# yoshitomo-matsubara/sc2-benchmark

Hardware: AMD Instinct MI355X
Metric: images/s + bpp, Entropic-Student ResNet-50 224^2 (higher is better)
Workload: dtype bf16

## Files before the change

### sc2-benchmark_amd/csrc/conv1x1_pair.hip

```cpp
#include <stdlib.h>

#include <atomic>

#include "sc2_common.h"

#ifndef SC2_NT_PAIR
#define SC2_NT_PAIR 0
#endif

namespace {

typedef __attribute__((address_space(3))) void *lds_ptr_t;
typedef float f32x2_t __attribute__((ext_vector_type(2)));
typedef __bf16 bf16x2_t __attribute__((ext_vector_type(2)));
typedef unsigned u32x4_t __attribute__((ext_vector_type(4)));
__device__ __forceinline__ uint32_t pack2(f32x2_t v) {
    return __builtin_bit_cast(uint32_t, __builtin_convertvector(v, bf16x2_t));
}

#if defined(__HIP_DEVICE_COMPILE__)
typedef __amdgpu_buffer_rsrc_t buf_rsrc_t;
__device__ __forceinline__ buf_rsrc_t make_rsrc(const uint16_t *base, uint32_t bytes) {
    return __builtin_amdgcn_make_buffer_rsrc(const_cast<uint16_t *>(base), 0, (int)bytes, 0x00020000);
}
__device__ __forceinline__ void buf_load_lds16(buf_rsrc_t r, lds_ptr_t dst, uint32_t voff, uint32_t soff) {
    __builtin_amdgcn_raw_ptr_buffer_load_lds(r, dst, 16, (int)voff, (int)soff, 0, 0);
}
__device__ __forceinline__ uint4 buf_load16(buf_rsrc_t r, uint32_t voff, uint32_t soff) {
    return __builtin_bit_cast(uint4, __builtin_amdgcn_raw_buffer_load_b128(r, (int)voff, (int)soff, 0));
}
__device__ __forceinline__ void buf_store16(buf_rsrc_t r, uint32_t voff, uint32_t soff, u32x4_t v) {
    __builtin_amdgcn_raw_buffer_store_b128(v, r, (int)voff, (int)soff, SC2_NT_PAIR ? SC2_BUF_AUX_NT : 0);
    __builtin_amdgcn_sched_barrier(0);
    asm volatile("s_nop 1" ::: "memory");
    __builtin_amdgcn_sched_barrier(0);
}
#else
typedef int buf_rsrc_t;
__device__ __forceinline__ buf_rsrc_t make_rsrc(const uint16_t *, uint32_t) { return 0; }
__device__ __forceinline__ void buf_load_lds16(buf_rsrc_t, lds_ptr_t, uint32_t, uint32_t) {}
__device__ __forceinline__ uint4 buf_load16(buf_rsrc_t, uint32_t, uint32_t) { return make_uint4(0, 0, 0, 0); }
__device__ __forceinline__ void buf_store16(buf_rsrc_t, uint32_t, uint32_t, u32x4_t) {}
#endif

template <int OFF>
__device__ __forceinline__ u32x4_t lds_read16_imm(uint32_t addr) {
    u32x4_t v;
    asm volatile("ds_read_b128 %0, %1 offset:%2" : "=v"(v) : "v"(addr), "n"(OFF) : "memory");
    return v;
}
__device__ __forceinline__ void lds_write16(uint32_t addr, u32x4_t v) {
    asm volatile("ds_write_b128 %0, %1" ::"v"(addr), "v"(v) : "memory");
}

#ifndef SC2_PAIR_DBG
#define SC2_PAIR_DBG 0
#endif

struct PairArgs {
    const uint16_t *__restrict__ o;
    const uint16_t *__restrict__ w3;
    const float *__restrict__ b3;
    const uint16_t *__restrict__ idn;
    uint16_t *__restrict__ h;
    const uint16_t *__restrict__ w1;
    const float *__restrict__ b1;
    uint16_t *__restrict__ u;
    int M, n_tiles;
    int rev;
    unsigned *tile_ctr;
};

template <int C, int K1, int N2, int MT>
__global__ __launch_bounds__(512, 2) void conv1x1_pair_kernel(const PairArgs p) {
    constexpr int P = MT * 16;
    constexpr int KS1 = K1 / 32, KS2 = C / 32;
    constexpr int NT1 = C / 8 / 16;
    constexpr int ROWB = C * 2;
    constexpr int CPR = ROWB / 16;
    constexpr int IMG = P * ROWB, SLAB = P * 64, OT = KS1 * SLAB;
    constexpr int NT2 = N2 / 128;
    static_assert(N2 == 128 || N2 == 256, "one or two 16-channel tiles of u per wave");
    static_assert(N2 <= C, "the u staging lives in the image region");
    static_assert(CPR == 64, "one image row = one LDS-DMA wave-instruction");
    constexpr int UROW = N2 * 2, UCPR = UROW / 16;
    constexpr int OQ = (P * K1 * 2 / 16 + 511) / 512;
    constexpr int UQ = (P * UCPR + 511) / 512;
    constexpr int IQ = (P * CPR + 511) / 512;
    extern __shared__ __attribute__((aligned(16))) unsigned char smem[];
    unsigned char *img = smem;
    unsigned char *ot = smem + IMG;
    volatile int *next_slot = reinterpret_cast<volatile int *>(smem + IMG + OT);
    float *bias_lds = reinterpret_cast<float *>(smem + IMG + OT + 16);

    const uint32_t lds_base = (uint32_t)(uintptr_t)(lds_ptr_t)smem;
    const int tid = threadIdx.x, lane = tid & 63;
    const int wn = __builtin_amdgcn_readfirstlane(tid >> 6);

    constexpr uint32_t OOB = 0x80000000u;
    const buf_rsrc_t rs_idn = make_rsrc(p.idn, (uint32_t)((long long)p.M * ROWB));
    const buf_rsrc_t rs_o = make_rsrc(p.o, (uint32_t)((long long)p.M * K1 * 2));
    const buf_rsrc_t rs_h = make_rsrc(p.h, (uint32_t)((long long)p.M * ROWB));
    const buf_rsrc_t rs_u = make_rsrc(p.u, (uint32_t)((long long)p.M * N2 * 2));

    auto load_o = [&](int tile, uint4 (&ov)[OQ], int tq) {
        const bool t_ok = tile < p.n_tiles;
        const int tpos = p.rev ? p.n_tiles - 1 - tile : tile;
        const uint32_t so = (uint32_t)(t_ok ? (long long)tpos * P * (K1 * 2) : 0);
#pragma unroll
        for (int k = 0; k < OQ; ++k) {
            const int q = tq + 512 * k;
            const bool ok = t_ok && q < P * (K1 / 8) && (long long)tpos * P + q / (K1 / 8) < p.M;
            ov[k] = buf_load16(rs_o, ok ? (uint32_t)q * 16u : OOB, so);
        }
    };
    auto store_o = [&](const uint4 (&ov)[OQ], int tq) {
#pragma unroll
        for (int k = 0; k < OQ; ++k) {
            const int q = tq + 512 * k;
            if (q < P * (K1 / 8)) {
                const int row = q / (K1 / 8), c16 = q % (K1 / 8);
                lds_write16(lds_base + IMG + (c16 >> 2) * SLAB + row * 64 + (((c16 & 3) ^ ((row >> 1) & 3)) << 4),
                            __builtin_bit_cast(u32x4_t, ov[k]));
            }
        }
    };
    auto issue_identity = [&](int tile, int lq) {
        static_assert(P % 8 == 0, "every wave takes P / 8 rows: straight-line issue, exact vmcnt bookkeeping");
#pragma unroll
        for (int r = 0; r < P / 8; ++r) {
            const int row = wn + 8 * r;
            const long long m = (long long)(p.rev ? p.n_tiles - 1 - tile : tile) * P + row;
            const bool ok = tile < p.n_tiles && m < p.M && !(SC2_PAIR_DBG & 1);
            const uint32_t voff = ok ? (uint32_t)((lq ^ (row & 15)) << 4) : OOB;
            buf_load_lds16(rs_idn, (lds_ptr_t)(img + row * ROWB), voff, (uint32_t)(ok ? m * ROWB : 0));
        }
    };

    uint4 wv[KS1][NT1];
    const buf_rsrc_t rs_w3 = make_rsrc(p.w3, (uint32_t)(C * K1 * 2));
    const uint32_t w3_vo = (uint32_t)(((wn * NT1) * KS1 * 64 + lane) * 16);
    auto load_w = [&]() {
#pragma unroll
        for (int j = 0; j < NT1; ++j)
#pragma unroll
            for (int s = 0; s < KS1; ++s) wv[s][j] = buf_load16(rs_w3, w3_vo, (uint32_t)((j * KS1 + s) * 1024));
    };
    load_w();
    const buf_rsrc_t rs_w1 = make_rsrc(p.w1, (uint32_t)(N2 * C * 2));
    const uint32_t w1_vo = (uint32_t)(((wn * NT2) * KS2 * 64 + lane) * 16);

    for (int k = tid; k < C + N2; k += 512) bias_lds[k] = k < C ? p.b3[k] : p.b1[k - C];
    int tile = blockIdx.x;
    int next_tile = tile + gridDim.x;
    {
        uint4 ov[OQ];
        load_o(tile, ov, tid);
        store_o(ov, tid);
        issue_identity(tile, lane);
    }
    __syncthreads();

    bool first = true;
    while (tile < p.n_tiles) {
        const long long m0 = (long long)(p.rev ? p.n_tiles - 1 - tile : tile) * P;
        int tq = tid, lq = lane;
        asm volatile("" : "+v"(tq), "+v"(lq));
        const int frow = lq & 15, fq = lq >> 4;
        const int o_lane = frow * 64 + ((fq ^ ((frow >> 1) & 3)) << 4);
        const int img_row = frow * ROWB;
        unsigned claimed = 0;
        if (tid == 0) {
            const unsigned one = 1u;
            asm volatile("global_atomic_add %0, %1, %2, off sc0" : "=v"(claimed) : "v"(p.tile_ctr), "v"(one) : "memory");
        }
        f32x4_t acc[MT][NT1];
#pragma unroll
        for (int i = 0; i < MT; ++i)
#pragma unroll
            for (int j = 0; j < NT1; ++j) acc[i][j] = f32x4_t{0.f, 0.f, 0.f, 0.f};
        {
            const uint32_t o_addr = lds_base + IMG + o_lane;
#pragma unroll
            for (int s = 0; s < KS1; ++s) {
                u32x4_t xa[4], xb[3];
                static_assert(MT == 7, "the asm waits below name 4 + 3 registers");
                xa[0] = lds_read16_imm<0 * 1024>(o_addr + s * SLAB);
                xa[1] = lds_read16_imm<1 * 1024>(o_addr + s * SLAB);
                xa[2] = lds_read16_imm<2 * 1024>(o_addr + s * SLAB);
                xa[3] = lds_read16_imm<3 * 1024>(o_addr + s * SLAB);
                asm volatile("s_waitcnt lgkmcnt(0)" : "+v"(xa[0]), "+v"(xa[1]), "+v"(xa[2]), "+v"(xa[3])::"memory");
                xb[0] = lds_read16_imm<4 * 1024>(o_addr + s * SLAB);
                xb[1] = lds_read16_imm<5 * 1024>(o_addr + s * SLAB);
                xb[2] = lds_read16_imm<6 * 1024>(o_addr + s * SLAB);
#pragma unroll
                for (int i = 0; i < 4; ++i) {
                    const bf16x8_t xf = __builtin_bit_cast(bf16x8_t, xa[i]);
#pragma unroll
                    for (int j = 0; j < NT1; ++j)
                        acc[i][j] = __builtin_amdgcn_mfma_f32_16x16x32_bf16(__builtin_bit_cast(bf16x8_t, wv[s][j]), xf, acc[i][j], 0, 0, 0);
                }
                asm volatile("s_waitcnt lgkmcnt(0)" : "+v"(xb[0]), "+v"(xb[1]), "+v"(xb[2])::"memory");
#pragma unroll
                for (int i = 0; i < 3; ++i) {
                    const bf16x8_t xf = __builtin_bit_cast(bf16x8_t, xb[i]);
#pragma unroll
                    for (int j = 0; j < NT1; ++j)
                        acc[4 + i][j] = __builtin_amdgcn_mfma_f32_16x16x32_bf16(__builtin_bit_cast(bf16x8_t, wv[s][j]), xf, acc[4 + i][j], 0, 0, 0);
                }
                __builtin_amdgcn_sched_barrier(0);
            }
        }
        if (first) asm volatile("s_waitcnt vmcnt(0)" ::: "memory");
        else if (wn == 0) asm volatile("s_waitcnt vmcnt(%0)" ::"n"(IQ + UQ + 1) : "memory");
        else asm volatile("s_waitcnt vmcnt(%0)" ::"n"(IQ + UQ) : "memory");
        first = false;
        __syncthreads();
#pragma unroll
        for (int j = 0; j < NT1; ++j) {
            const int c16 = wn * (NT1 * 2) + j * 2 + (fq >> 1);
            const float4 b3v = *reinterpret_cast<const float4 *>(bias_lds + wn * (NT1 * 16) + j * 16 + fq * 4);
            const f32x2_t b01 = {b3v.x, b3v.y}, b23 = {b3v.z, b3v.w};
            const int slot_lane = img_row + ((c16 ^ frow) << 4) + (fq & 1) * 8;
#pragma unroll
            for (int i = 0; i < MT; ++i) {
                unsigned char *slot = img + slot_lane + i * (16 * ROWB);
                const uint2 xr = *reinterpret_cast<const uint2 *>(slot);
                f32x2_t v01 = f32x2_t{acc[i][j][0], acc[i][j][1]} + b01;
                f32x2_t v23 = f32x2_t{acc[i][j][2], acc[i][j][3]} + b23;
                v01 += f32x2_t{__builtin_bit_cast(float, xr.x << 16), __builtin_bit_cast(float, xr.x & 0xFFFF0000u)};
                v23 += f32x2_t{__builtin_bit_cast(float, xr.y << 16), __builtin_bit_cast(float, xr.y & 0xFFFF0000u)};
                v01 = f32x2_t{fmaxf(v01[0], 0.f), fmaxf(v01[1], 0.f)};
                v23 = f32x2_t{fmaxf(v23[0], 0.f), fmaxf(v23[1], 0.f)};
                uint2 o2;
                o2.x = pack2(v01);
                o2.y = pack2(v23);
                *reinterpret_cast<uint2 *>(slot) = o2;
                if ((i & 3) == 3) __builtin_amdgcn_sched_barrier(0);
            }
        }
        __syncthreads();
        __builtin_amdgcn_sched_barrier(0);
        constexpr int GB = 8;
        uint4 gb[GB][NT2];
#pragma unroll
        for (int ks = 0; ks < GB; ++ks)
#pragma unroll
            for (int t = 0; t < NT2; ++t) gb[ks][t] = buf_load16(rs_w1, w1_vo, (uint32_t)((t * KS2 + ks) * 1024));
        uint4 ov[OQ];
        load_o(next_tile, ov, tq);
        f32x4_t acc2[MT][NT2];
#pragma unroll
        for (int i = 0; i < MT; ++i)
#pragma unroll
            for (int t = 0; t < NT2; ++t) acc2[i][t] = f32x4_t{0.f, 0.f, 0.f, 0.f};
#pragma unroll
        for (int ks = 0; ks < ((SC2_PAIR_DBG & 4) ? 0 : KS2); ++ks) {
            bf16x8_t gf[NT2];
#pragma unroll
            for (int t = 0; t < NT2; ++t) {
                gf[t] = __builtin_bit_cast(bf16x8_t, gb[ks % GB][t]);
                if (ks + GB < KS2) gb[ks % GB][t] = buf_load16(rs_w1, w1_vo, (uint32_t)((t * KS2 + ks + GB) * 1024));
            }
            const int rd_lane = img_row + (((ks * 4 + fq) ^ frow) << 4);
#pragma unroll
            for (int i = 0; i < MT; ++i) {
                const bf16x8_t xf = __builtin_bit_cast(bf16x8_t, *reinterpret_cast<const uint4 *>(img + rd_lane + i * (16 * ROWB)));
#pragma unroll
                for (int t = 0; t < NT2; ++t) acc2[i][t] = __builtin_amdgcn_mfma_f32_16x16x32_bf16(gf[t], xf, acc2[i][t], 0, 0, 0);
            }
            if ((ks & 1) == 1) __builtin_amdgcn_sched_barrier(0);
        }
        if (tid == 0) {
            asm volatile("s_waitcnt vmcnt(%1)" : "+v"(claimed) : "n"(OQ) : "memory");
            *next_slot = (int)(claimed + 2 * gridDim.x);
            if (claimed == (unsigned)(p.n_tiles - 1)) *p.tile_ctr = 0u;
        }
        u32x4_t hv[IQ];
#pragma unroll
        for (int k = 0; k < IQ; ++k) {
            const int q = tq + 512 * k;
            const int row = q / CPR, c = q % CPR;
            hv[k] = *reinterpret_cast<const u32x4_t *>(img + row * ROWB + ((c ^ (row & 15)) << 4));
        }
        __syncthreads();
        store_o(ov, tq);
#pragma unroll
        for (int t = 0; t < NT2; ++t) {
            const float4 b1v = *reinterpret_cast<const float4 *>(bias_lds + C + (wn * NT2 + t) * 16 + fq * 4);
            const f32x2_t b01 = {b1v.x, b1v.y}, b23 = {b1v.z, b1v.w};
            const int c16 = (wn * NT2 + t) * 2 + (fq >> 1);
            const int u_lane = frow * UROW + ((c16 ^ frow) << 4) + (fq & 1) * 8;
#pragma unroll
            for (int i = 0; i < MT; ++i) {
                f32x2_t v01 = f32x2_t{acc2[i][t][0], acc2[i][t][1]} + b01;
                f32x2_t v23 = f32x2_t{acc2[i][t][2], acc2[i][t][3]} + b23;
                v01 = f32x2_t{fmaxf(v01[0], 0.f), fmaxf(v01[1], 0.f)};
                v23 = f32x2_t{fmaxf(v23[0], 0.f), fmaxf(v23[1], 0.f)};
                uint2 o2;
                o2.x = pack2(v01);
                o2.y = pack2(v23);
                *reinterpret_cast<uint2 *>(img + u_lane + i * (16 * UROW)) = o2;
            }
        }
        asm volatile("s_waitcnt lgkmcnt(0)" ::: "memory");
        __syncthreads();
        const int tile_after_next = __builtin_amdgcn_readfirstlane(*next_slot);
        u32x4_t uv[UQ];
#pragma unroll
        for (int k = 0; k < UQ; ++k) {
            const int q = tq + 512 * k;
            const int row = q / UCPR, c = q % UCPR;
            const int qq = q < P * UCPR ? row * UROW + ((c ^ (row & 15)) << 4) : 0;
            uv[k] = *reinterpret_cast<const u32x4_t *>(img + qq);
        }
        __syncthreads();
        issue_identity(next_tile, lq);
        {
            const uint32_t so = (uint32_t)(m0 * ROWB);
#pragma unroll
            for (int k = 0; k < IQ; ++k) {
                const int q = tq + 512 * k;
                buf_store16(rs_h, (q < P * CPR && m0 + q / CPR < p.M && !(SC2_PAIR_DBG & 2)) ? (uint32_t)q * 16u : OOB, so, hv[k]);
            }
        }
        {
            const uint32_t so = (uint32_t)(m0 * UROW);
#pragma unroll
            for (int k = 0; k < UQ; ++k) {
                const int q = tq + 512 * k;
                buf_store16(rs_u, (q < P * UCPR && m0 + q / UCPR < p.M && !(SC2_PAIR_DBG & 2)) ? (uint32_t)q * 16u : OOB, so, uv[k]);
            }
        }
        tile = next_tile;
        next_tile = tile_after_next;
    }
}

constexpr int kRing = 256;
sc2_counter_ring g_ring;
std::atomic<unsigned> g_seq{0};

template <int C, int K1, int N2, int MT>
int launch_pair(const PairArgs &a, hipStream_t s) {
    constexpr int P = MT * 16;
    constexpr int lds = P * C * 2 + (K1 / 32) * P * 64 + 16 + (C + N2) * 4;
    static_assert(lds <= 160 * 1024, "image + o tile must fit the CU's LDS");
    static bool attr_set[SC2_MAX_DEVICES] = {};
    const int dev = sc2_device_slot();
    if (!attr_set[dev]) {
        (void)hipFuncSetAttribute(reinterpret_cast<const void *>(&conv1x1_pair_kernel<C, K1, N2, MT>),
                                  hipFuncAttributeMaxDynamicSharedMemorySize, lds);
        attr_set[dev] = true;
    }
    const int g_cus = sc2_device_cus();
    unsigned *slot = g_ring.launch_slot(s, kRing, 1, g_seq);
    if (!slot) return SC2_ERR_INTERNAL;
    PairArgs b = a;
    b.n_tiles = (a.M + P - 1) / P;
    b.tile_ctr = slot;
    {
        const int alt = sc2_pol().pair_alt;
        static std::atomic<unsigned> calls{0};
        b.rev = alt ? (int)(calls.fetch_add(1) & 1u) : 0;
    }
    const int grid = b.n_tiles < g_cus ? b.n_tiles : g_cus;
    hipLaunchKernelGGL((conv1x1_pair_kernel<C, K1, N2, MT>), dim3(grid), dim3(512), lds, s, b);
    SC2_CHECK_LAUNCH();
    return SC2_OK;
}

}

extern "C" int sc2_conv1x1_pair_supported(int K1, int C, int N2) { return (K1 == 128 && C == 512 && (N2 == 128 || N2 == 256)) ? 1 : 0; }

extern "C" int sc2_conv1x1_pair_fwd(const void *o, const void *w3_frag, const float *b3, const void *identity, void *h,
                                    const void *w1_frag, const float *b1, void *u, long long M, int K1, int C, int N2,
                                    void *stream) {
    SC2_REQUIRE(o && w3_frag && b3 && identity && h && w1_frag && b1 && u, SC2_ERR_INVALID_ARG, "conv1x1_pair: null argument");
    SC2_REQUIRE(sc2_conv1x1_pair_supported(K1, C, N2), SC2_ERR_UNSUPPORTED, "conv1x1_pair: K1 %d C %d N2 %d not supported", K1, C, N2);
    SC2_REQUIRE(M > 0 && M * C * 2 < 0x7FF00000LL, SC2_ERR_UNSUPPORTED, "conv1x1_pair: M = %lld outside the 32-bit buffer range", M);
    PairArgs a;
    a.o = static_cast<const uint16_t *>(o); a.w3 = static_cast<const uint16_t *>(w3_frag); a.b3 = b3;
    a.idn = static_cast<const uint16_t *>(identity); a.h = static_cast<uint16_t *>(h);
    a.w1 = static_cast<const uint16_t *>(w1_frag); a.b1 = b1; a.u = static_cast<uint16_t *>(u);
    a.M = (int)M; a.n_tiles = 0; a.tile_ctr = nullptr; a.rev = 0;
    if (N2 == 256) return launch_pair<512, 128, 256, 7>(a, static_cast<hipStream_t>(stream));
    return launch_pair<512, 128, 128, 7>(a, static_cast<hipStream_t>(stream));
}
```

### sc2-benchmark_amd/csrc/conv1x1_stream.hip

```cpp
#include <stdlib.h>

#include <atomic>

#include <type_traits>

#include "sc2_common.h"

#ifndef SC2_STREAM_EARLY
#define SC2_STREAM_EARLY 1
#endif
#ifndef SC2_NT_STREAM
#define SC2_NT_STREAM 0
#endif

namespace {

struct StreamArgs {
    const uint16_t *__restrict__ x;
    const uint16_t *__restrict__ w;
    const float *__restrict__ bias;
    const uint16_t *__restrict__ res;
    uint16_t *__restrict__ y;
    const uint16_t *__restrict__ mask;
    int H, W, OH, OW, OHW, M, Cout, stride, relu;
    int n_chunks, n_units;
    unsigned *unit_ctr;
};


typedef float f32x2_t __attribute__((ext_vector_type(2)));
typedef unsigned u32x4_t __attribute__((ext_vector_type(4)));
typedef __bf16 bf16x2_t __attribute__((ext_vector_type(2)));
__device__ __forceinline__ uint32_t pack2(f32x2_t v) {
    return __builtin_bit_cast(uint32_t, __builtin_convertvector(v, bf16x2_t));
}

template <int K, int BM, int BNC, bool RES, bool MASK = false>
__global__ __launch_bounds__(512, 2) void conv1x1_stream_kernel(const StreamArgs p) {
    constexpr int MT = BM / 16, NT = BNC / 16 / 8;
    constexpr int CPI = BNC / 8;
    constexpr int KS = K / 32;
    constexpr int A_BYTES = BM * K * 2;
    constexpr int CPR = K / 8;
    constexpr int A_Q = BM * CPR / 512;
    constexpr int IMG_Q = BM * CPI / 512;
    constexpr int ASW = CPR >= 16 ? 15 : CPR - 1;
    extern __shared__ __attribute__((aligned(16))) unsigned char smem[];
    __shared__ int next_slot;
    unsigned char *At = smem;
    unsigned char *img = smem + A_BYTES;

    const int tid = threadIdx.x;
    const int lane = tid & 63;
    const int wn = __builtin_amdgcn_readfirstlane(tid >> 6);
    const int frow = lane & 15, fq = lane >> 4;
    const int Cout = p.Cout;

    u32x4_t a_next[A_Q], r_next[RES ? IMG_Q : 1];
    uint4 w_regs[KS][NT];
    float4 b_next[NT];

    auto load_unit = [&](int unit, int tid, auto part_c) {
        constexpr int PART = decltype(part_c)::value;
        const bool live = unit < p.n_units;
        const int tile = live ? unit / p.n_chunks : 0;
        const int chunk = live ? unit - tile * p.n_chunks : 0;
        const int m0 = tile * BM;
        if (PART != 1) {
#pragma unroll
            for (int j = 0; j < NT; ++j)
                b_next[j] = *reinterpret_cast<const float4 *>(p.bias + chunk * BNC + wn * (NT * 16) + j * 16 + ((tid & 63) >> 4) * 4);
        }
        if (PART == 2) return;
        const uint4 *wf = reinterpret_cast<const uint4 *>(p.w) + ((long long)(chunk * (BNC / 16) + wn * NT) * KS) * 64 + (tid & 63);
#pragma unroll
        for (int j = 0; j < NT; ++j)
#pragma unroll
            for (int ks = 0; ks < KS; ++ks) w_regs[ks][j] = wf[(j * KS + ks) * 64];
        if (RES) {
#pragma unroll
            for (int k = 0; k < IMG_Q; ++k) {
                const int q = tid + 512 * k;
                const int row = q / CPI, c = q % CPI;
                const int m = min(m0 + row, p.M - 1);
                r_next[k] = *reinterpret_cast<const u32x4_t *>(p.res + (long long)m * Cout + chunk * BNC + c * 8);
            }
        }
        if (p.stride != 1) {
#pragma unroll
            for (int k = 0; k < A_Q; ++k) {
                const int q = tid + 512 * k;
                const int row = q / CPR, c = q - row * CPR;
                const int m = min(m0 + row, p.M - 1);
                const int im = m / p.OHW, rem = m - im * p.OHW;
                const int oh = rem / p.OW, ow = rem - oh * p.OW;
                const long long pix = ((long long)im * p.H + oh * p.stride) * p.W + ow * p.stride;
                a_next[k] = *reinterpret_cast<const u32x4_t *>(p.x + pix * K + c * 8);
            }
        } else {
#pragma unroll
            for (int k = 0; k < A_Q; ++k) {
                const int q = tid + 512 * k;
                const int row = q / CPR, c = q - row * CPR;
                const long long pix = min(m0 + row, p.M - 1);
                a_next[k] = *reinterpret_cast<const u32x4_t *>(p.x + pix * K + c * 8);
            }
        }
    };
    auto store_a = [&](int tid) {
#pragma unroll
        for (int k = 0; k < A_Q; ++k) {
            const int q = tid + 512 * k;
            const int row = q / CPR, c = q - row * CPR;
            *reinterpret_cast<u32x4_t *>(At + row * (K * 2) + ((c ^ (row & ASW)) << 4)) = a_next[k];
        }
    };

    int unit = blockIdx.x;
    int next_unit = unit + gridDim.x;
    load_unit(unit, tid, std::integral_constant<int, 0>{});
    store_a(tid);
    __syncthreads();

    while (unit < p.n_units) {
        const int tile = unit / p.n_chunks;
        const int chunk = unit - tile * p.n_chunks;
        const int m0 = tile * BM;

        f32x4_t acc[MT][NT];
#pragma unroll
        for (int i = 0; i < MT; ++i)
#pragma unroll
            for (int j = 0; j < NT; ++j) acc[i][j] = f32x4_t{0.f, 0.f, 0.f, 0.f};
#pragma unroll
        for (int ks = 0; ks < KS; ++ks) {
            const int a_lane = frow * (K * 2) + (((ks * 4 + fq) ^ (frow & ASW)) << 4);
#pragma unroll
            for (int i = 0; i < MT; ++i) {
                const bf16x8_t af = __builtin_bit_cast(bf16x8_t, *reinterpret_cast<const uint4 *>(At + a_lane + i * 16 * K * 2));
#pragma unroll
                for (int j = 0; j < NT; ++j)
                    acc[i][j] = __builtin_amdgcn_mfma_f32_16x16x32_bf16(__builtin_bit_cast(bf16x8_t, w_regs[ks][j]), af,
                                                                        acc[i][j], 0, 0, 0);
            }
        }
        if (RES) {
#pragma unroll
            for (int k = 0; k < IMG_Q; ++k) {
                const int q = tid + 512 * k;
                const int row = q / CPI, c = q % CPI;
                *reinterpret_cast<u32x4_t *>(img + row * (BNC * 2) + ((c ^ (row & 15)) << 4)) = r_next[k];
            }
        }
        constexpr bool EARLY = SC2_STREAM_EARLY && !(K == 512 && BNC == 256 && RES);
        if (EARLY) load_unit(next_unit, tid, std::integral_constant<int, 1>{});
        __syncthreads();
        auto finish = [&](auto relu_c) {
            constexpr bool RELU = decltype(relu_c)::value;
#pragma unroll
            for (int j = 0; j < NT; ++j) {
                const int col = wn * (NT * 16) + j * 16 + fq * 4;
                const float4 b4 = b_next[j];
                const f32x2_t b01 = {b4.x, b4.y}, b23 = {b4.z, b4.w};
#pragma unroll
                for (int i = 0; i < MT; ++i) {
                    const int row = i * 16 + frow;
                    unsigned char *slot = img + row * (BNC * 2) + (((col >> 3) ^ frow) << 4) + (col & 7) * 2;
                    f32x2_t v01 = f32x2_t{acc[i][j][0], acc[i][j][1]} + b01;
                    f32x2_t v23 = f32x2_t{acc[i][j][2], acc[i][j][3]} + b23;
                    if (RES) {
                        const uint2 xr = *reinterpret_cast<const uint2 *>(slot);
                        v01 += f32x2_t{__builtin_bit_cast(float, xr.x << 16), __builtin_bit_cast(float, xr.x & 0xFFFF0000u)};
                        v23 += f32x2_t{__builtin_bit_cast(float, xr.y << 16), __builtin_bit_cast(float, xr.y & 0xFFFF0000u)};
                    }
                    if (RELU) {
                        v01 = f32x2_t{fmaxf(v01[0], 0.f), fmaxf(v01[1], 0.f)};
                        v23 = f32x2_t{fmaxf(v23[0], 0.f), fmaxf(v23[1], 0.f)};
                    }
                    uint2 o;
                    o.x = pack2(v01);
                    o.y = pack2(v23);
                    *reinterpret_cast<uint2 *>(slot) = o;
                }
            }
        };
        if (p.relu) finish(std::true_type{});
        else finish(std::false_type{});
        __syncthreads();
        int tq = tid;
        asm volatile("" : "+v"(tq));
        unsigned claimed = 0;
        if (tid == 0) {
            const unsigned one = 1u;
            asm volatile("global_atomic_add %0, %1, %2, off sc0" : "=v"(claimed) : "v"(p.unit_ctr), "v"(one) : "memory");
        }
        if (EARLY) load_unit(next_unit, tq, std::integral_constant<int, 2>{});
        else load_unit(next_unit, tq, std::integral_constant<int, 0>{});
        {
            uint4 *yo = reinterpret_cast<uint4 *>(p.y + (long long)chunk * BNC);
            [[maybe_unused]] uint4 mq[MASK ? IMG_Q : 1];
            if constexpr (MASK) {
                const uint4 *mo = reinterpret_cast<const uint4 *>(p.mask + (long long)chunk * BNC);
#pragma unroll
                for (int k = 0; k < IMG_Q; ++k) {
                    const int q = tq + 512 * k;
                    int row = q / CPI;
                    const int c = q % CPI;
                    row = m0 + row < p.M ? row : 0;
                    mq[k] = mo[(long long)(m0 + row) * (Cout / 8) + c];
                }
            }
#pragma unroll
            for (int k = 0; k < IMG_Q; ++k) {
                const int q = tq + 512 * k;
                int row = q / CPI;
                const int c = q % CPI;
                row = m0 + row < p.M ? row : 0;
                uint4 ov = *reinterpret_cast<const uint4 *>(img + row * (BNC * 2) + ((c ^ (row & 15)) << 4));
                if constexpr (MASK) {
                    const uint32_t mw[4] = {mq[k].x, mq[k].y, mq[k].z, mq[k].w};
                    uint32_t ow[4] = {ov.x, ov.y, ov.z, ov.w};
#pragma unroll
                    for (int e = 0; e < 4; ++e)
                        ow[e] = (__builtin_bit_cast(float, mw[e] << 16) > 0.f ? ow[e] & 0xFFFFu : 0u) |
                                (__builtin_bit_cast(float, mw[e] & 0xFFFF0000u) > 0.f ? ow[e] & 0xFFFF0000u : 0u);
                    ov = make_uint4(ow[0], ow[1], ow[2], ow[3]);
                }
                if (SC2_NT_STREAM) sc2_store16_nt(yo + (long long)(m0 + row) * (Cout / 8) + c, ov);
                else yo[(long long)(m0 + row) * (Cout / 8) + c] = ov;
            }
        }
        store_a(tq);
        if (tid == 0) {
            asm volatile("s_waitcnt vmcnt(%1)" : "+v"(claimed) : "n"(IMG_Q) : "memory");
            next_slot = (int)(claimed + 2 * gridDim.x);
            if (claimed == (unsigned)(p.n_units - 1)) *p.unit_ctr = 0u;
        }
        __syncthreads();
        unit = next_unit;
        next_unit = __builtin_amdgcn_readfirstlane(next_slot);
    }
}

constexpr int kRing = 256;
sc2_counter_ring g_ring;
std::atomic<unsigned> g_seq{0};

template <int K, int BM, int BNC, bool RES, bool MASK = false>
int launch_stream(const StreamArgs &a0, hipStream_t s) {
    constexpr int lds = BM * K * 2 + BM * BNC * 2;
    StreamArgs a = a0;
    a.n_chunks = a.Cout / BNC;
    const long long units = (((long long)a.M + BM - 1) / BM) * a.n_chunks;
    if (units >= 0x7FFFFFFFLL - 1024) {
        sc2_set_error("conv1x1_stream: too many units");
        return SC2_ERR_UNSUPPORTED;
    }
    a.n_units = (int)units;
    static bool attr_set_dev[SC2_MAX_DEVICES] = {};
    bool &attr_set = attr_set_dev[sc2_device_slot()];
    if (!attr_set) {
        (void)hipFuncSetAttribute(reinterpret_cast<const void *>(&conv1x1_stream_kernel<K, BM, BNC, RES, MASK>),
                                  hipFuncAttributeMaxDynamicSharedMemorySize, lds);
        attr_set = true;
    }
    const int g_cus = sc2_device_cus();
    unsigned *slot = g_ring.launch_slot(s, kRing, 1, g_seq);
    if (!slot) return SC2_ERR_INTERNAL;
    static sc2_per_device_int per_cu_dev;
    int per_cu = per_cu_dev.here().load(std::memory_order_relaxed);
    if (per_cu == 0) {
        int n = 0;
        if (hipOccupancyMaxActiveBlocksPerMultiprocessor(&n, reinterpret_cast<const void *>(&conv1x1_stream_kernel<K, BM, BNC, RES, MASK>), 512,
                                                         lds) != hipSuccess || n < 1)
            n = 1;
        per_cu = n > 2 ? 2 : n;
        per_cu_dev.here().store(per_cu, std::memory_order_relaxed);
    }
    const int slots = g_cus * per_cu;
    const int grid = a.n_units < slots ? a.n_units : slots;
    StreamArgs b = a;
    b.unit_ctr = slot;
    hipLaunchKernelGGL((conv1x1_stream_kernel<K, BM, BNC, RES, MASK>), dim3(grid), dim3(512), lds, s, b);
    SC2_CHECK_LAUNCH();
    return SC2_OK;
}

}

extern "C" int sc2_conv1x1_stream_supported(int Cin, int Cout, int stride) {
    return (Cin == 64 || Cin == 128 || Cin == 256 || Cin == 512) && Cout >= 128 && Cout % 128 == 0 && (stride == 1 || stride == 2) ? 1 : 0;
}

extern "C" int sc2_conv1x1_stream_mask_supported(int Cin, int Cout, int stride) {
    return (Cin == 128 || Cin == 256) && Cout % 256 == 0 && Cout >= 256 && stride == 1 ? 1 : 0;
}

extern "C" int sc2_conv1x1_stream_fwd(const void *x, const void *w_frag, const float *bias, const void *residual, const void *mask,
                                      void *y, int N, int H, int W, int Cin, int Cout, int stride, int relu, void *stream) {
    SC2_REQUIRE(x && w_frag && bias && y, SC2_ERR_INVALID_ARG, "conv1x1_stream: null argument");
    SC2_REQUIRE(!mask || (!relu && sc2_conv1x1_stream_mask_supported(Cin, Cout, stride)), SC2_ERR_UNSUPPORTED,
                "conv1x1_stream: the mask form needs Cin 128 / 256, Cout %% 256 == 0, stride 1, no relu (got %d -> %d, stride %d)", Cin, Cout,
                stride);
    SC2_REQUIRE(N > 0 && H > 0 && W > 0, SC2_ERR_INVALID_ARG, "conv1x1_stream: non-positive dimension");
    SC2_REQUIRE(sc2_conv1x1_stream_supported(Cin, Cout, stride), SC2_ERR_UNSUPPORTED,
                "conv1x1_stream: needs Cin in {64, 128, 256, 512}, Cout %% 128 == 0, stride 1 or 2 (got %d -> %d, stride %d)", Cin,
                Cout, stride);
    StreamArgs a;
    a.x = static_cast<const uint16_t *>(x);
    a.w = static_cast<const uint16_t *>(w_frag);
    a.bias = bias;
    a.res = static_cast<const uint16_t *>(residual);
    a.mask = static_cast<const uint16_t *>(mask);
    a.y = static_cast<uint16_t *>(y);
    a.H = H; a.W = W;
    a.OH = (H - 1) / stride + 1;
    a.OW = (W - 1) / stride + 1;
    a.OHW = a.OH * a.OW;
    const long long M = (long long)N * a.OHW;
    SC2_REQUIRE(M < 0x7FFFFFFFLL - 256, SC2_ERR_UNSUPPORTED, "conv1x1_stream: N*OH*OW = %lld exceeds 2^31", M);
    a.M = (int)M; a.Cout = Cout; a.stride = stride; a.relu = relu ? 1 : 0;
    a.n_chunks = 0; a.n_units = 0;
    a.unit_ctr = nullptr;
    hipStream_t s = static_cast<hipStream_t>(stream);
    if (a.mask) {
        if (Cin == 128) return a.res ? launch_stream<128, 128, 256, true, true>(a, s) : launch_stream<128, 128, 256, false, true>(a, s);
        return a.res ? launch_stream<256, 128, 256, true, true>(a, s) : launch_stream<256, 128, 256, false, true>(a, s);
    }
#define SC2_STREAM_GO(KK, BMM, BNN) return a.res ? launch_stream<KK, BMM, BNN, true>(a, s) : launch_stream<KK, BMM, BNN, false>(a, s)
    if (Cin == 512 && Cout % 256 == 0) SC2_STREAM_GO(512, 64, 256);
    if (Cin == 512) SC2_STREAM_GO(512, 64, 128);
    if (Cin == 64 && Cout % 256 == 0) SC2_STREAM_GO(64, 128, 256);
    if (Cin == 64) SC2_STREAM_GO(64, 128, 128);
    if (Cout % 256 == 0) {
        if (Cin == 128) SC2_STREAM_GO(128, 128, 256);
        SC2_STREAM_GO(256, 128, 256);
    }
    if (Cin == 128) SC2_STREAM_GO(128, 128, 128);
    SC2_STREAM_GO(256, 128, 128);
#undef SC2_STREAM_GO
}
```

Before: 45300.

## Add small-tile two-workgroup-per-CU form of fused 1x1 conv pair for N2=128

Adds an MT=3 variant of the fused conv1x1 pair kernel, now the default for N2=128. Phase 1 runs in two halves over output channels to cut accumulator registers, and w3 weights are reloaded each tile instead of held for the kernel's lifetime. Launch bounds allow four waves per SIMD, and the grid is sized from queried occupancy so two workgroups can share a CU. This trades extra weight reloads and smaller tiles for higher occupancy and latency hiding, and it adds a debug flag that skips the atomic tile counter.

```diff
diff --git a/sc2-benchmark_amd/csrc/conv1x1_pair.hip b/sc2-benchmark_amd/csrc/conv1x1_pair.hip
--- a/sc2-benchmark_amd/csrc/conv1x1_pair.hip
+++ b/sc2-benchmark_amd/csrc/conv1x1_pair.hip
@@ -55,6 +55,14 @@
 
 #ifndef SC2_PAIR_DBG
 #define SC2_PAIR_DBG 0
+#endif
+
+#ifdef SC2_PAIR_MT
+#define SC2_PAIR_MT_128 SC2_PAIR_MT
+#define SC2_PAIR_MT_256 SC2_PAIR_MT
+#else
+#define SC2_PAIR_MT_128 3
+#define SC2_PAIR_MT_256 7
 #endif
 
 struct PairArgs {
@@ -72,10 +80,16 @@
 };
 
 template <int C, int K1, int N2, int MT>
-__global__ __launch_bounds__(512, 2) void conv1x1_pair_kernel(const PairArgs p) {
+__global__ __launch_bounds__(512, MT <= 3 ? 4 : 2) void conv1x1_pair_kernel(const PairArgs p) {
+    static_assert(MT == 7 || MT == 3, "the fragment batches of phase 1 and the read-ahead depths are written out for these two");
+    constexpr bool W3_STREAM = MT <= 3;
+    constexpr int NH = W3_STREAM ? 2 : 1;
     constexpr int P = MT * 16;
     constexpr int KS1 = K1 / 32, KS2 = C / 32;
     constexpr int NT1 = C / 8 / 16;
+    constexpr int NTH = NT1 / NH;
+    constexpr bool W3_LATE = W3_STREAM && N2 == 256;
+    constexpr int WQ = W3_LATE ? NTH * (K1 / 32) : 0;
     constexpr int ROWB = C * 2;
     constexpr int CPR = ROWB / 16;
     constexpr int IMG = P * ROWB, SLAB = P * 64, OT = KS1 * SLAB;
@@ -140,13 +154,13 @@
     uint4 wv[KS1][NT1];
     const buf_rsrc_t rs_w3 = make_rsrc(p.w3, (uint32_t)(C * K1 * 2));
     const uint32_t w3_vo = (uint32_t)(((wn * NT1) * KS1 * 64 + lane) * 16);
-    auto load_w = [&]() {
-#pragma unroll
-        for (int j = 0; j < NT1; ++j)
+    auto load_w = [&](int j0, int j1) {
+#pragma unroll
+        for (int j = j0; j < j1; ++j)
 #pragma unroll
             for (int s = 0; s < KS1; ++s) wv[s][j] = buf_load16(rs_w3, w3_vo, (uint32_t)((j * KS1 + s) * 1024));
     };
-    load_w();
+    load_w(0, W3_LATE ? NTH : NT1);
     const buf_rsrc_t rs_w1 = make_rsrc(p.w1, (uint32_t)(N2 * C * 2));
     const uint32_t w1_vo = (uint32_t)(((wn * NT2) * KS2 * 64 + lane) * 16);
 
@@ -170,21 +184,24 @@
         const int o_lane = frow * 64 + ((fq ^ ((frow >> 1) & 3)) << 4);
         const int img_row = frow * ROWB;
         unsigned claimed = 0;
-        if (tid == 0) {
+        if (tid == 0 && !(SC2_PAIR_DBG & 8)) {
             const unsigned one = 1u;
             asm volatile("global_atomic_add %0, %1, %2, off sc0" : "=v"(claimed) : "v"(p.tile_ctr), "v"(one) : "memory");
         }
-        f32x4_t acc[MT][NT1];
+        if constexpr (W3_LATE) load_w(NTH, NT1);
+#pragma unroll
+        for (int hf = 0; hf < NH; ++hf) {
+        f32x4_t acc[MT][NTH];
 #pragma unroll
         for (int i = 0; i < MT; ++i)
 #pragma unroll
-            for (int j = 0; j < NT1; ++j) acc[i][j] = f32x4_t{0.f, 0.f, 0.f, 0.f};
+            for (int j = 0; j < NTH; ++j) acc[i][j] = f32x4_t{0.f, 0.f, 0.f, 0.f};
         {
             const uint32_t o_addr = lds_base + IMG + o_lane;
 #pragma unroll
             for (int s = 0; s < KS1; ++s) {
+                if constexpr (MT == 7) {
                 u32x4_t xa[4], xb[3];
-                static_assert(MT == 7, "the asm waits below name 4 + 3 registers");
                 xa[0] = lds_read16_imm<0 * 1024>(o_addr + s * SLAB);
                 xa[1] = lds_read16_imm<1 * 1024>(o_addr + s * SLAB);
                 xa[2] = lds_read16_imm<2 * 1024>(o_addr + s * SLAB);
@@ -197,27 +214,44 @@
                 for (int i = 0; i < 4; ++i) {
                     const bf16x8_t xf = __builtin_bit_cast(bf16x8_t, xa[i]);
 #pragma unroll
-                    for (int j = 0; j < NT1; ++j)
-                        acc[i][j] = __builtin_amdgcn_mfma_f32_16x16x32_bf16(__builtin_bit_cast(bf16x8_t, wv[s][j]), xf, acc[i][j], 0, 0, 0);
+                    for (int j = 0; j < NTH; ++j)
+                        acc[i][j] = __builtin_amdgcn_mfma_f32_16x16x32_bf16(__builtin_bit_cast(bf16x8_t, wv[s][hf * NTH + j]), xf, acc[i][j], 0, 0, 0);
                 }
                 asm volatile("s_waitcnt lgkmcnt(0)" : "+v"(xb[0]), "+v"(xb[1]), "+v"(xb[2])::"memory");
 #pragma unroll
                 for (int i = 0; i < 3; ++i) {
                     const bf16x8_t xf = __builtin_bit_cast(bf16x8_t, xb[i]);
 #pragma unroll
-                    for (int j = 0; j < NT1; ++j)
-                        acc[4 + i][j] = __builtin_amdgcn_mfma_f32_16x16x32_bf16(__builtin_bit_cast(bf16x8_t, wv[s][j]), xf, acc[4 + i][j], 0, 0, 0);
+                    for (int j = 0; j < NTH; ++j)
+                        acc[4 + i][j] = __builtin_amdgcn_mfma_f32_16x16x32_bf16(__builtin_bit_cast(bf16x8_t, wv[s][hf * NTH + j]), xf, acc[4 + i][j], 0, 0, 0);
+                }
+                } else {
+                u32x4_t xa[3];
+                xa[0] = lds_read16_imm<0 * 1024>(o_addr + s * SLAB);
+                xa[1] = lds_read16_imm<1 * 1024>(o_addr + s * SLAB);
+                xa[2] = lds_read16_imm<2 * 1024>(o_addr + s * SLAB);
+                asm volatile("s_waitcnt lgkmcnt(0)" : "+v"(xa[0]), "+v"(xa[1]), "+v"(xa[2])::"memory");
+#pragma unroll
+                for (int i = 0; i < 3; ++i) {
+                    const bf16x8_t xf = __builtin_bit_cast(bf16x8_t, xa[i]);
+#pragma unroll
+                    for (int j = 0; j < NTH; ++j)
+                        acc[i][j] = __builtin_amdgcn_mfma_f32_16x16x32_bf16(__builtin_bit_cast(bf16x8_t, wv[s][hf * NTH + j]), xf, acc[i][j], 0, 0, 0);
+                }
                 }
                 __builtin_amdgcn_sched_barrier(0);
             }
         }
+        if (hf == 0) {
         if (first) asm volatile("s_waitcnt vmcnt(0)" ::: "memory");
-        else if (wn == 0) asm volatile("s_waitcnt vmcnt(%0)" ::"n"(IQ + UQ + 1) : "memory");
-        else asm volatile("s_waitcnt vmcnt(%0)" ::"n"(IQ + UQ) : "memory");
+        else if (wn == 0) asm volatile("s_waitcnt vmcnt(%0)" ::"n"(IQ + UQ + WQ + 1) : "memory");
+        else asm volatile("s_waitcnt vmcnt(%0)" ::"n"(IQ + UQ + WQ) : "memory");
         first = false;
         __syncthreads();
-#pragma unroll
-        for (int j = 0; j < NT1; ++j) {
+        }
+#pragma unroll
+        for (int jh = 0; jh < NTH; ++jh) {
+            const int j = hf * NTH + jh;
             const int c16 = wn * (NT1 * 2) + j * 2 + (fq >> 1);
             const float4 b3v = *reinterpret_cast<const float4 *>(bias_lds + wn * (NT1 * 16) + j * 16 + fq * 4);
             const f32x2_t b01 = {b3v.x, b3v.y}, b23 = {b3v.z, b3v.w};
@@ -226,8 +260,8 @@
             for (int i = 0; i < MT; ++i) {
                 unsigned char *slot = img + slot_lane + i * (16 * ROWB);
                 const uint2 xr = *reinterpret_cast<const uint2 *>(slot);
-                f32x2_t v01 = f32x2_t{acc[i][j][0], acc[i][j][1]} + b01;
-                f32x2_t v23 = f32x2_t{acc[i][j][2], acc[i][j][3]} + b23;
+                f32x2_t v01 = f32x2_t{acc[i][jh][0], acc[i][jh][1]} + b01;
+                f32x2_t v23 = f32x2_t{acc[i][jh][2], acc[i][jh][3]} + b23;
                 v01 += f32x2_t{__builtin_bit_cast(float, xr.x << 16), __builtin_bit_cast(float, xr.x & 0xFFFF0000u)};
                 v23 += f32x2_t{__builtin_bit_cast(float, xr.y << 16), __builtin_bit_cast(float, xr.y & 0xFFFF0000u)};
                 v01 = f32x2_t{fmaxf(v01[0], 0.f), fmaxf(v01[1], 0.f)};
@@ -239,9 +273,10 @@
                 if ((i & 3) == 3) __builtin_amdgcn_sched_barrier(0);
             }
         }
+        }
         __syncthreads();
         __builtin_amdgcn_sched_barrier(0);
-        constexpr int GB = 8;
+        constexpr int GB = (W3_STREAM && NT2 == 1) ? KS2 : (W3_STREAM ? 6 : 8);
         uint4 gb[GB][NT2];
 #pragma unroll
         for (int ks = 0; ks < GB; ++ks)
@@ -271,7 +306,9 @@
             }
             if ((ks & 1) == 1) __builtin_amdgcn_sched_barrier(0);
         }
-        if (tid == 0) {
+        if (SC2_PAIR_DBG & 8) {
+            if (tid == 0) *next_slot = next_tile + (int)gridDim.x;
+        } else if (tid == 0) {
             asm volatile("s_waitcnt vmcnt(%1)" : "+v"(claimed) : "n"(OQ) : "memory");
             *next_slot = (int)(claimed + 2 * gridDim.x);
             if (claimed == (unsigned)(p.n_tiles - 1)) *p.tile_ctr = 0u;
@@ -315,6 +352,7 @@
             uv[k] = *reinterpret_cast<const u32x4_t *>(img + qq);
         }
         __syncthreads();
+        if constexpr (W3_STREAM) load_w(0, W3_LATE ? NTH : NT1);
         issue_identity(next_tile, lq);
         {
             const uint32_t so = (uint32_t)(m0 * ROWB);
@@ -346,6 +384,7 @@
     constexpr int P = MT * 16;
     constexpr int lds = P * C * 2 + (K1 / 32) * P * 64 + 16 + (C + N2) * 4;
     static_assert(lds <= 160 * 1024, "image + o tile must fit the CU's LDS");
+    static_assert(MT > 3 || 2 * lds <= 160 * 1024, "the small form runs two workgroups per CU");
     static bool attr_set[SC2_MAX_DEVICES] = {};
     const int dev = sc2_device_slot();
     if (!attr_set[dev]) {
@@ -364,7 +403,18 @@
         static std::atomic<unsigned> calls{0};
         b.rev = alt ? (int)(calls.fetch_add(1) & 1u) : 0;
     }
-    const int grid = b.n_tiles < g_cus ? b.n_tiles : g_cus;
+    static sc2_per_device_int per_cu_dev;
+    int per_cu = per_cu_dev.here().load(std::memory_order_relaxed);
+    if (per_cu == 0) {
+        int n = 0;
+        if (hipOccupancyMaxActiveBlocksPerMultiprocessor(&n, reinterpret_cast<const void *>(&conv1x1_pair_kernel<C, K1, N2, MT>), 512,
+                                                         lds) != hipSuccess || n < 1)
+            n = 1;
+        per_cu = n > 2 ? 2 : n;
+        per_cu_dev.here().store(per_cu, std::memory_order_relaxed);
+    }
+    const int slots = g_cus * per_cu;
+    const int grid = b.n_tiles < slots ? b.n_tiles : slots;
     hipLaunchKernelGGL((conv1x1_pair_kernel<C, K1, N2, MT>), dim3(grid), dim3(512), lds, s, b);
     SC2_CHECK_LAUNCH();
     return SC2_OK;
@@ -385,6 +435,6 @@
     a.idn = static_cast<const uint16_t *>(identity); a.h = static_cast<uint16_t *>(h);
     a.w1 = static_cast<const uint16_t *>(w1_frag); a.b1 = b1; a.u = static_cast<uint16_t *>(u);
     a.M = (int)M; a.n_tiles = 0; a.tile_ctr = nullptr; a.rev = 0;
-    if (N2 == 256) return launch_pair<512, 128, 256, 7>(a, static_cast<hipStream_t>(stream));
-    return launch_pair<512, 128, 128, 7>(a, static_cast<hipStream_t>(stream));
-}
+    if (N2 == 256) return launch_pair<512, 128, 256, SC2_PAIR_MT_256>(a, static_cast<hipStream_t>(stream));
+    return launch_pair<512, 128, 128, SC2_PAIR_MT_128>(a, static_cast<hipStream_t>(stream));
+}
```

Result: no change. 45210 (-0.2%).

## Pin output-channel chunk per block and add 112-row tiles for better wave quantization

Applied to the files above, without the earlier changes.

Adds a FIXED mode in which each persistent block owns one output-channel chunk. Weights and bias are then loaded once instead of per unit, and per-chunk atomic counters are used. It also adds a BM=112 tile variant, chosen on the host when it gives fewer wasted rows across persistent rounds, with the A buffer padded so every thread moves equal chunks. This reduces repeated weight register loads and tail imbalance, at the cost of more template instantiations and a query path through the API.

```diff
diff --git a/sc2-benchmark_amd/csrc/conv1x1_stream.hip b/sc2-benchmark_amd/csrc/conv1x1_stream.hip
--- a/sc2-benchmark_amd/csrc/conv1x1_stream.hip
+++ b/sc2-benchmark_amd/csrc/conv1x1_stream.hip
@@ -8,6 +8,12 @@
 
 #ifndef SC2_STREAM_EARLY
 #define SC2_STREAM_EARLY 1
+#endif
+#ifndef SC2_STREAM_BM112
+#define SC2_STREAM_BM112 1
+#endif
+#ifndef SC2_STREAM_FIXED
+#define SC2_STREAM_FIXED 1
 #endif
 #ifndef SC2_NT_STREAM
 #define SC2_NT_STREAM 0
@@ -28,6 +34,9 @@
 };
 
 
+constexpr int stream_a_rows(int K, int BM) { return (BM * (K / 8) + 511) / 512 * 512 / (K / 8); }
+constexpr int stream_lds_bytes(int K, int BM, int BNC) { return stream_a_rows(K, BM) * K * 2 + BM * BNC * 2; }
+
 typedef float f32x2_t __attribute__((ext_vector_type(2)));
 typedef unsigned u32x4_t __attribute__((ext_vector_type(4)));
 typedef __bf16 bf16x2_t __attribute__((ext_vector_type(2)));
@@ -35,15 +44,19 @@
     return __builtin_bit_cast(uint32_t, __builtin_convertvector(v, bf16x2_t));
 }
 
-template <int K, int BM, int BNC, bool RES, bool MASK = false>
+template <int K, int BM, int BNC, bool RES, bool MASK = false, bool FIXED = false>
 __global__ __launch_bounds__(512, 2) void conv1x1_stream_kernel(const StreamArgs p) {
     constexpr int MT = BM / 16, NT = BNC / 16 / 8;
     constexpr int CPI = BNC / 8;
     constexpr int KS = K / 32;
-    constexpr int A_BYTES = BM * K * 2;
+    constexpr int A_ROWS = stream_a_rows(K, BM);
+    constexpr int A_BYTES = A_ROWS * K * 2;
     constexpr int CPR = K / 8;
-    constexpr int A_Q = BM * CPR / 512;
+    constexpr int A_Q = A_ROWS * CPR / 512;
     constexpr int IMG_Q = BM * CPI / 512;
+    static_assert(BM % 16 == 0 && BNC % 128 == 0, "whole MFMA tiles per wave");
+    static_assert(A_ROWS >= BM && A_ROWS * CPR == A_Q * 512, "every thread moves the same number of A chunks");
+    static_assert(BM * CPI == IMG_Q * 512, "every thread moves the same number of image chunks");
     constexpr int ASW = CPR >= 16 ? 15 : CPR - 1;
     extern __shared__ __attribute__((aligned(16))) unsigned char smem[];
     __shared__ int next_slot;
@@ -60,23 +73,30 @@
     uint4 w_regs[KS][NT];
     float4 b_next[NT];
 
+    const int my_chunk = FIXED ? (int)(blockIdx.x % (unsigned)p.n_chunks) : 0;
+    const int grp_idx = FIXED ? (int)(blockIdx.x / (unsigned)p.n_chunks) : (int)blockIdx.x;
+    const int grp_size = FIXED ? (int)(gridDim.x / (unsigned)p.n_chunks) : (int)gridDim.x;
+
     auto load_unit = [&](int unit, int tid, auto part_c) {
         constexpr int PART = decltype(part_c)::value;
+        constexpr bool WB = !FIXED || PART == 3;
         const bool live = unit < p.n_units;
-        const int tile = live ? unit / p.n_chunks : 0;
-        const int chunk = live ? unit - tile * p.n_chunks : 0;
+        const int tile = FIXED ? (live ? unit : 0) : live ? unit / p.n_chunks : 0;
+        const int chunk = FIXED ? my_chunk : live ? unit - tile * p.n_chunks : 0;
         const int m0 = tile * BM;
-        if (PART != 1) {
+        if (PART != 1 && WB) {
 #pragma unroll
             for (int j = 0; j < NT; ++j)
                 b_next[j] = *reinterpret_cast<const float4 *>(p.bias + chunk * BNC + wn * (NT * 16) + j * 16 + ((tid & 63) >> 4) * 4);
         }
         if (PART == 2) return;
-        const uint4 *wf = reinterpret_cast<const uint4 *>(p.w) + ((long long)(chunk * (BNC / 16) + wn * NT) * KS) * 64 + (tid & 63);
-#pragma unroll
-        for (int j = 0; j < NT; ++j)
-#pragma unroll
-            for (int ks = 0; ks < KS; ++ks) w_regs[ks][j] = wf[(j * KS + ks) * 64];
+        if (WB) {
+            const uint4 *wf = reinterpret_cast<const uint4 *>(p.w) + ((long long)(chunk * (BNC / 16) + wn * NT) * KS) * 64 + (tid & 63);
+#pragma unroll
+            for (int j = 0; j < NT; ++j)
+#pragma unroll
+                for (int ks = 0; ks < KS; ++ks) w_regs[ks][j] = wf[(j * KS + ks) * 64];
+        }
         if (RES) {
 #pragma unroll
             for (int k = 0; k < IMG_Q; ++k) {
@@ -116,15 +136,15 @@
         }
     };
 
-    int unit = blockIdx.x;
-    int next_unit = unit + gridDim.x;
-    load_unit(unit, tid, std::integral_constant<int, 0>{});
+    int unit = grp_idx;
+    int next_unit = unit + grp_size;
+    load_unit(unit, tid, std::integral_constant<int, 3>{});
     store_a(tid);
     __syncthreads();
 
     while (unit < p.n_units) {
-        const int tile = unit / p.n_chunks;
-        const int chunk = unit - tile * p.n_chunks;
+        const int tile = FIXED ? unit : unit / p.n_chunks;
+        const int chunk = FIXED ? my_chunk : unit - tile * p.n_chunks;
         const int m0 = tile * BM;
 
         f32x4_t acc[MT][NT];
@@ -190,9 +210,10 @@
         int tq = tid;
         asm volatile("" : "+v"(tq));
         unsigned claimed = 0;
+        unsigned *const ctr = p.unit_ctr + my_chunk;
         if (tid == 0) {
             const unsigned one = 1u;
-            asm volatile("global_atomic_add %0, %1, %2, off sc0" : "=v"(claimed) : "v"(p.unit_ctr), "v"(one) : "memory");
+            asm volatile("global_atomic_add %0, %1, %2, off sc0" : "=v"(claimed) : "v"(ctr), "v"(one) : "memory");
         }
         if (EARLY) load_unit(next_unit, tq, std::integral_constant<int, 2>{});
         else load_unit(next_unit, tq, std::integral_constant<int, 0>{});
@@ -233,8 +254,8 @@
         store_a(tq);
         if (tid == 0) {
             asm volatile("s_waitcnt vmcnt(%1)" : "+v"(claimed) : "n"(IMG_Q) : "memory");
-            next_slot = (int)(claimed + 2 * gridDim.x);
-            if (claimed == (unsigned)(p.n_units - 1)) *p.unit_ctr = 0u;
+            next_slot = (int)(claimed + 2 * grp_size);
+            if (claimed == (unsigned)(p.n_units - 1)) *ctr = 0u;
         }
         __syncthreads();
         unit = next_unit;
@@ -242,50 +263,77 @@
     }
 }
 
-constexpr int kRing = 256;
+constexpr int kCtrs = 8;
+constexpr int kRing = 256 * kCtrs;
 sc2_counter_ring g_ring;
 std::atomic<unsigned> g_seq{0};
 
-template <int K, int BM, int BNC, bool RES, bool MASK = false>
-int launch_stream(const StreamArgs &a0, hipStream_t s) {
-    constexpr int lds = BM * K * 2 + BM * BNC * 2;
-    StreamArgs a = a0;
-    a.n_chunks = a.Cout / BNC;
-    const long long units = (((long long)a.M + BM - 1) / BM) * a.n_chunks;
-    if (units >= 0x7FFFFFFFLL - 1024) {
-        sc2_set_error("conv1x1_stream: too many units");
-        return SC2_ERR_UNSUPPORTED;
-    }
-    a.n_units = (int)units;
+template <int K, int BM, int BNC, bool RES, bool MASK = false, bool FIXED = false>
+int stream_slots() {
+    constexpr int lds = stream_lds_bytes(K, BM, BNC);
     static bool attr_set_dev[SC2_MAX_DEVICES] = {};
     bool &attr_set = attr_set_dev[sc2_device_slot()];
     if (!attr_set) {
-        (void)hipFuncSetAttribute(reinterpret_cast<const void *>(&conv1x1_stream_kernel<K, BM, BNC, RES, MASK>),
+        (void)hipFuncSetAttribute(reinterpret_cast<const void *>(&conv1x1_stream_kernel<K, BM, BNC, RES, MASK, FIXED>),
                                   hipFuncAttributeMaxDynamicSharedMemorySize, lds);
         attr_set = true;
     }
-    const int g_cus = sc2_device_cus();
-    unsigned *slot = g_ring.launch_slot(s, kRing, 1, g_seq);
-    if (!slot) return SC2_ERR_INTERNAL;
     static sc2_per_device_int per_cu_dev;
     int per_cu = per_cu_dev.here().load(std::memory_order_relaxed);
     if (per_cu == 0) {
         int n = 0;
-        if (hipOccupancyMaxActiveBlocksPerMultiprocessor(&n, reinterpret_cast<const void *>(&conv1x1_stream_kernel<K, BM, BNC, RES, MASK>), 512,
-                                                         lds) != hipSuccess || n < 1)
+        if (hipOccupancyMaxActiveBlocksPerMultiprocessor(&n, reinterpret_cast<const void *>(&conv1x1_stream_kernel<K, BM, BNC, RES, MASK, FIXED>),
+                                                         512, lds) != hipSuccess || n < 1)
             n = 1;
         per_cu = n > 2 ? 2 : n;
         per_cu_dev.here().store(per_cu, std::memory_order_relaxed);
     }
-    const int slots = g_cus * per_cu;
+    return sc2_device_cus() * per_cu;
+}
+
+template <int K, int BM, int BNC, bool RES, bool MASK = false>
+int launch_stream(const StreamArgs &a0, hipStream_t s) {
+    constexpr int lds = stream_lds_bytes(K, BM, BNC);
+    StreamArgs a = a0;
+    a.n_chunks = a.Cout / BNC;
+    const long long tiles = ((long long)a.M + BM - 1) / BM, units = tiles * a.n_chunks;
+    if (units >= 0x7FFFFFFFLL - 1024) {
+        sc2_set_error("conv1x1_stream: too many units");
+        return SC2_ERR_UNSUPPORTED;
+    }
+    a.n_units = (int)units;
+    unsigned *slot = g_ring.launch_slot(s, kRing, kCtrs, g_seq);
+    if (!slot) return SC2_ERR_INTERNAL;
+    a.unit_ctr = slot;
+    if constexpr (SC2_STREAM_FIXED && BNC == 256 && (K == 128 || K == 256 || (K == 512 && !RES)) && !MASK) {
+        const int slots = stream_slots<K, BM, BNC, RES, MASK, true>();
+        const int grid = a.n_units < slots ? a.n_units : slots;
+        if (a.n_chunks <= kCtrs && grid % a.n_chunks == 0) {
+            a.n_units = (int)tiles;
+            hipLaunchKernelGGL((conv1x1_stream_kernel<K, BM, BNC, RES, MASK, true>), dim3(grid), dim3(512), lds, s, a);
+            SC2_CHECK_LAUNCH();
+            return SC2_OK;
+        }
+    }
+    const int slots = stream_slots<K, BM, BNC, RES, MASK>();
     const int grid = a.n_units < slots ? a.n_units : slots;
-    StreamArgs b = a;
-    b.unit_ctr = slot;
-    hipLaunchKernelGGL((conv1x1_stream_kernel<K, BM, BNC, RES, MASK>), dim3(grid), dim3(512), lds, s, b);
+    hipLaunchKernelGGL((conv1x1_stream_kernel<K, BM, BNC, RES, MASK>), dim3(grid), dim3(512), lds, s, a);
     SC2_CHECK_LAUNCH();
     return SC2_OK;
 }
 
+template <int K, bool RES>
+int stream_unit_pixels(int M, int Cout) {
+#if SC2_STREAM_BM112
+    const long long chunks = Cout / 256;
+    const long long s128 = stream_slots<K, 128, 256, RES>(), s112 = stream_slots<K, 112, 256, RES>();
+    const long long u128 = ((long long)M + 127) / 128 * chunks, u112 = ((long long)M + 111) / 112 * chunks;
+    return (u112 + s112 - 1) / s112 * 112 < (u128 + s128 - 1) / s128 * 128 ? 112 : 128;
+#else
+    return 128;
+#endif
+}
+
 }
 
 extern "C" int sc2_conv1x1_stream_supported(int Cin, int Cout, int stride) {
@@ -298,7 +346,8 @@
 
 extern "C" int sc2_conv1x1_stream_fwd(const void *x, const void *w_frag, const float *bias, const void *residual, const void *mask,
                                       void *y, int N, int H, int W, int Cin, int Cout, int stride, int relu, void *stream) {
-    SC2_REQUIRE(x && w_frag && bias && y, SC2_ERR_INVALID_ARG, "conv1x1_stream: null argument");
+    const bool query = !x && !w_frag && !bias && !y;
+    SC2_REQUIRE(query || (x && w_frag && bias && y), SC2_ERR_INVALID_ARG, "conv1x1_stream: null argument");
     SC2_REQUIRE(!mask || (!relu && sc2_conv1x1_stream_mask_supported(Cin, Cout, stride)), SC2_ERR_UNSUPPORTED,
                 "conv1x1_stream: the mask form needs Cin 128 / 256, Cout %% 256 == 0, stride 1, no relu (got %d -> %d, stride %d)", Cin, Cout,
                 stride);
@@ -323,6 +372,13 @@
     a.n_chunks = 0; a.n_units = 0;
     a.unit_ctr = nullptr;
     hipStream_t s = static_cast<hipStream_t>(stream);
+    const bool rounds = !a.mask && (Cin == 128 || Cin == 256) && Cout % 256 == 0;
+    int bm = Cin == 512 ? 64 : 128;
+    if (rounds) {
+        if (Cin == 128) bm = residual ? stream_unit_pixels<128, true>(a.M, Cout) : stream_unit_pixels<128, false>(a.M, Cout);
+        else bm = residual ? stream_unit_pixels<256, true>(a.M, Cout) : stream_unit_pixels<256, false>(a.M, Cout);
+    }
+    if (query) return bm;
     if (a.mask) {
         if (Cin == 128) return a.res ? launch_stream<128, 128, 256, true, true>(a, s) : launch_stream<128, 128, 256, false, true>(a, s);
         return a.res ? launch_stream<256, 128, 256, true, true>(a, s) : launch_stream<256, 128, 256, false, true>(a, s);
@@ -333,7 +389,9 @@
     if (Cin == 64 && Cout % 256 == 0) SC2_STREAM_GO(64, 128, 256);
     if (Cin == 64) SC2_STREAM_GO(64, 128, 128);
     if (Cout % 256 == 0) {
+        if (Cin == 128 && bm == 112) SC2_STREAM_GO(128, 112, 256);
         if (Cin == 128) SC2_STREAM_GO(128, 128, 256);
+        if (bm == 112) SC2_STREAM_GO(256, 112, 256);
         SC2_STREAM_GO(256, 128, 256);
     }
     if (Cin == 128) SC2_STREAM_GO(128, 128, 128);
```

Result: no change. 45300 before, 45720 after (median of 6 runs) (+0.9%).
